# mvisionai/PyGrid

Hardware: AMD Instinct MI355X
Metric: client-diff GB/s aggregated (% of HBM peak) at 1/2/4/8 MI355X; cycle close ms (higher is better)
Workload: dtype f32; 1 GPU; resnet18-fedavg: P_shard=11689512 params/GPU x 1000 clients fp32, resident in HBM; clients=1000, params_per_gpu=11689512, params_total=11689512, parallelism=param-shard1, kernel_variant=0

## Files before the change

### pygrid_amd/csrc/pgh_api.cpp

```cpp
#include <sched.h>

#include <fstream>

#include "pgh_ctx.h"

namespace pgh_detail {

std::vector<int> gpu_local_cpus(int device) {
    std::vector<int> out;
    char bus[64] = {0};
    if (hipDeviceGetPCIBusId(bus, sizeof bus, device) != hipSuccess) { (void)hipGetLastError(); return out; }
    std::string id(bus);
    for (auto& ch : id) ch = (char)std::tolower((unsigned char)ch);
    std::ifstream f("/sys/bus/pci/devices/" + id + "/local_cpulist");
    std::string list;
    if (!f || !std::getline(f, list)) return out;
    cpu_set_t allowed;
    CPU_ZERO(&allowed);
    if (sched_getaffinity(0, sizeof allowed, &allowed) != 0) return out;
    size_t pos = 0;
    while (pos < list.size()) {
        size_t end = list.find(',', pos);
        if (end == std::string::npos) end = list.size();
        const std::string r = list.substr(pos, end - pos);
// ... 105 lines not shown
    *nb = (pg + b - 1) / b;
    int sh = 0;
    while ((int64_t(1) << sh) < b) ++sh;
    *bshift = sh;
}

}

using namespace pgh_detail;

extern "C" {

int pgh_abi_version(void) { return PGH_ABI_VERSION; }

int pgh_device_count(int* n) {
    if (!n) return PGH_E_ARG;
    int k = 0;
    hipError_t e = hipGetDeviceCount(&k);
    if (e != hipSuccess) { *n = 0; return fail(nullptr, PGH_E_HIP, "hipGetDeviceCount: %s", hipGetErrorString(e)); }
    *n = k;
    return PGH_OK;
}

const char* pgh_last_error(const pgh_ctx* ctx) { return ctx ? ctx->err.c_str() : g_create_err.c_str(); }

int pgh_create(int device, size_t pinned_bytes, pgh_ctx** out) {
    if (!out) return fail(nullptr, PGH_E_ARG, "out is NULL");
    *out = nullptr;
    int ndev = 0;
    hipError_t e = hipGetDeviceCount(&ndev);
    if (e != hipSuccess || ndev <= 0) return fail(nullptr, PGH_E_HIP, "no HIP device: %s", hipGetErrorString(e));
    if (device < 0 || device >= ndev) return fail(nullptr, PGH_E_ARG, "device %d out of range [0,%d)", device, ndev);
    auto* c = new pgh_ctx();
    c->device = device;
    DeviceGuard g(device);
    if (pinned_bytes == 0) pinned_bytes = 256ull << 20;
    c->ring.slot_bytes = (pinned_bytes / 2) & ~(size_t)4095;
    if (c->ring.slot_bytes < 4096) c->ring.slot_bytes = 4096;
    c->copy_threads = std::min(16, pgh_int::usable_cpus());
    if (const char* e = std::getenv("PGH_COPY_THREADS")) c->copy_threads = std::max(1, std::atoi(e));
    {
        const char* nu = std::getenv("PGH_NUMA");
        if (!nu || std::atoi(nu) != 0) c->local_cpus = gpu_local_cpus(device);
    }
    c->pool_copy.reset(new CopyPool(c->copy_threads, c->local_cpus));
    if (const char* e = std::getenv("PGH_BLOCK_BYTES")) c->block_bytes = (size_t)std::max(0LL, std::atoll(e));
    if (const char* e = std::getenv("PGH_FINAL_RANGES")) c->final_split = std::max(1, std::atoi(e));
    bool ok = c->stream.make() == hipSuccess && c->copy.make() == hipSuccess && c->aux.make() == hipSuccess;
    ok = ok && xfer_made(c);
    for (pgh_ctx::Event* ev : {&c->copy_done, &c->xsync, &c->aux_ev}) ok = ok && ev->make() == hipSuccess;
    ok = ok && rules_made(c);
    if (!ok) { pgh_destroy(c); return fail(nullptr, PGH_E_HIP, "stream/event creation failed"); }
    {
        bool pin_ok = true;
        auto alloc = [&] {
            bind_thread(c->local_cpus);
            const unsigned flags = c->local_cpus.empty() ? hipHostMallocDefault : hipHostMallocNumaUser;
            for (int k = 0; k < 2 && pin_ok; ++k)
                pin_ok = c->ring.h_pin[k].reserve(c->ring.slot_bytes, flags) ||
                         (flags != hipHostMallocDefault && c->ring.h_pin[k].reserve(c->ring.slot_bytes));
        };
        if (c->local_cpus.empty()) alloc();
        else std::thread([&] { DeviceGuard g2(device); alloc(); }).join();
        if (!pin_ok) {
            const size_t bytes = c->ring.slot_bytes;
            pgh_destroy(c);
            return fail(nullptr, PGH_E_OOM, "pinned host allocation of %zu bytes failed", bytes);
        }
    }
    const char* wu = std::getenv("PGH_WARMUP");
    if (!wu || std::atoi(wu) != 0) {
        const int64_t n = (int64_t)std::min(c->ring.slot_bytes, (size_t)2 << 20) / 8;
        void* d = nullptr;
        ok = hipMalloc(&d, 12 * n) == hipSuccess;
        if (ok) {
            int64_t* d_sum = (int64_t*)d;
            float* d_dec = (float*)((uint8_t*)d + 8 * n);
            void* const pin0 = c->ring.h_pin[0].as<void>();
            std::memset(pin0, 0, 8 * n);
            ok = hipMemcpyAsync(d_sum, pin0, 8 * n, hipMemcpyHostToDevice, c->copy) == hipSuccess &&
                 hipStreamSynchronize(c->copy) == hipSuccess &&
                 (!c->d2h.s || (hipMemcpyAsync(d_sum, pin0, 8 * n, hipMemcpyHostToDevice, c->d2h.s) == hipSuccess &&
                                hipStreamSynchronize(c->d2h.s) == hipSuccess)) &&
                 pgh::launch_secagg_decode(d_sum, d_dec, n, 1.0f, c->stream) == hipSuccess &&
                 hipMemcpyAsync(c->ring.h_pin[1].as<void>(), d_sum, 8 * n, hipMemcpyDeviceToHost, c->stream) == hipSuccess &&
                 hipStreamSynchronize(c->stream) == hipSuccess;
            (void)hipFree(d);
        }
        if (!ok) {
            (void)hipGetLastError();
            (void)hipStreamSynchronize(c->copy);
            (void)hipStreamSynchronize(c->stream);
            c->warmup_skipped = true;
        }
    }
    *out = c;
    return PGH_OK;
}

void pgh_destroy(pgh_ctx* c) {
    if (!c) return;
    if (c->grp) { pgh_group_api::destroy(c); return; }
    DeviceGuard g(c->device);
    sync_work(c);
    if (c->d2h.s) (void)hipStreamSynchronize(c->d2h.s);
    delete c;
}

int pgh_set_layout(pgh_ctx* c, int n_tensors, const int64_t* numel) {
    if (c && c->grp) return pgh_group_api::set_layout(c, n_tensors, numel);
    if (!c) return PGH_E_ARG;
    if (n_tensors <= 0 || !numel) return fail(c, PGH_E_ARG, "need at least one tensor");
    int64_t P = 0;
    for (int k = 0; k < n_tensors; ++k) {
        if (numel[k] < 0) return fail(c, PGH_E_ARG, "tensor %d has negative numel", k);
        P += numel[k];
    }
    if (P <= 0) return fail(c, PGH_E_ARG, "model has no parameters");
    DeviceGuard g(c->device);
    free_slab(c);
    c->numel.assign(numel, numel + n_tensors);
    c->P = P;
    c->layout = true;
    return pgh_set_shard(c, 0, P);
}

int pgh_set_shard(pgh_ctx* c, int64_t lo, int64_t hi) {
    if (c && c->grp) return pgh_group_api::set_shard(c, lo, hi);
    if (!c) return PGH_E_ARG;
    return pgh_detail::set_shard(c, lo, hi, false);
}

}

int pgh_detail::set_shard(pgh_ctx* c, int64_t lo, int64_t hi, bool keep_opt) {
    if (!c->layout) return fail(c, PGH_E_STATE, "pgh_set_layout has not been called");
    if (lo < 0 || hi > c->P || lo >= hi)
        return fail(c, PGH_E_ARG, "shard [%lld,%lld) outside [0,%lld)", (long long)lo, (long long)hi, (long long)c->P);
    DeviceGuard g(c->device);
    free_slab(c);
    const int64_t pvec = std::max((hi - lo + 63) & ~(int64_t)63, (c->vec_min + 63) & ~(int64_t)63);
    rules_shard_set(c, lo, hi, pvec, keep_opt);
    c->lo = lo;
    c->hi = hi;
    c->pg = hi - lo;
    c->pvec = pvec;
    c->st.p_shard = c->pg;
    return PGH_OK;
// ... 184 lines not shown
```

### pygrid_amd/csrc/pgh_host.cpp

```cpp
#include "pgh_host.h"

#include <emmintrin.h>
#include <pthread.h>
#include <sched.h>
#include <sys/mman.h>
#include <unistd.h>

#include <cfloat>
#include <cmath>
#include <cstdlib>
#include <cstring>
#include <fstream>
#include <string>

namespace pgh_detail {

void copy_stream(uint8_t* dst, const uint8_t* src, size_t n) {
    if (n < (256u << 10)) { std::memcpy(dst, src, n); return; }
    const size_t head = (16 - (reinterpret_cast<uintptr_t>(dst) & 15)) & 15;
    std::memcpy(dst, src, head);
    dst += head; src += head; n -= head;
    size_t i = 0;
    for (; i + 64 <= n; i += 64) {
        const __m128i a = _mm_loadu_si128(reinterpret_cast<const __m128i*>(src + i));
        const __m128i b = _mm_loadu_si128(reinterpret_cast<const __m128i*>(src + i + 16));
        const __m128i c = _mm_loadu_si128(reinterpret_cast<const __m128i*>(src + i + 32));
        const __m128i d = _mm_loadu_si128(reinterpret_cast<const __m128i*>(src + i + 48));
        _mm_stream_si128(reinterpret_cast<__m128i*>(dst + i), a);
        _mm_stream_si128(reinterpret_cast<__m128i*>(dst + i + 16), b);
        _mm_stream_si128(reinterpret_cast<__m128i*>(dst + i + 32), c);
        _mm_stream_si128(reinterpret_cast<__m128i*>(dst + i + 48), d);
    }
    std::memcpy(dst + i, src + i, n - i);
    _mm_sfence();
}

void bind_thread(const std::vector<int>& cpus) {
    if (cpus.empty()) return;
    cpu_set_t set;
    CPU_ZERO(&set);
    for (int c : cpus)
        if (c >= 0 && c < CPU_SETSIZE) CPU_SET(c, &set);
    (void)pthread_setaffinity_np(pthread_self(), sizeof set, &set);
}

void scatter_out(const uint8_t* src, size_t off, size_t len, const std::vector<OutPiece>& pieces, CopyPool& pool) {
    std::vector<CopyPool::Seg> segs;
    size_t base = 0;
    for (auto& p : pieces) {
        const size_t a = std::max(off, base), b = std::min(off + len, base + p.n);
        if (a < b) segs.push_back({p.dst + (a - base), src + (a - off), b - a});
        base += p.n;
        if (base >= off + len) break;
    }
    pool.run(segs);
}

void prefault_small(uint8_t* p, size_t n) {
#ifndef MADV_POPULATE_WRITE
#define MADV_POPULATE_WRITE 23
#endif
    if (!p || n == 0 || n >= (4u << 20)) return;
    static const uintptr_t page = (uintptr_t)sysconf(_SC_PAGESIZE);
    const uintptr_t a = (uintptr_t)p & ~(page - 1), b = ((uintptr_t)p + n + page - 1) & ~(page - 1);
    (void)madvise((void*)a, b - a, MADV_POPULATE_WRITE);
}

void prefault_small_any(uint8_t* p, size_t n) {
    static const uintptr_t page = (uintptr_t)sysconf(_SC_PAGESIZE);
    const uintptr_t a = (uintptr_t)p & ~(page - 1), b = ((uintptr_t)p + n + page - 1) & ~(page - 1);
    (void)madvise((void*)a, b - a, MADV_POPULATE_WRITE);
}

bool all_resident(uintptr_t a, uintptr_t b, uintptr_t page) {
    std::vector<unsigned char> v((size_t)((b - a) / page));
    if (v.empty() || mincore((void*)a, b - a, v.data()) != 0) return false;
    for (unsigned char x : v)
        if (!(x & 1)) return false;
    return true;
}

void prefault_parallel(uint8_t* p, size_t n, CopyPool& pool) {
    if (!p || n == 0) return;
    if (n < (4u << 20)) { prefault_small(p, n); return; }
    static const uintptr_t page = (uintptr_t)sysconf(_SC_PAGESIZE);
    const uintptr_t a = (uintptr_t)p & ~(page - 1), b = ((uintptr_t)p + n + page - 1) & ~(page - 1);
    if (all_resident(a, b, page)) return;
    const int k = pool.threads();
    const uintptr_t per = ((b - a) / k + page - 1) & ~(page - 1);
    pool.run_items(k, true, [&](int i) {
        const uintptr_t lo = a + per * (uintptr_t)i, hi = std::min(b, lo + per);
        if (lo < hi) (void)madvise((void*)lo, hi - lo, MADV_POPULATE_WRITE);
    });
}


void philox4x32_10(const uint32_t ctr[4], const uint32_t key[2], uint32_t out[4]) {
    uint32_t c0 = ctr[0], c1 = ctr[1], c2 = ctr[2], c3 = ctr[3], k0 = key[0], k1 = key[1];
    for (int r = 0; r < 10; ++r) {
        const uint64_t p0 = (uint64_t)0xD2511F53u * c0, p1 = (uint64_t)0xCD9E8D57u * c2;
        const uint32_t n0 = (uint32_t)(p1 >> 32) ^ c1 ^ k0, n2 = (uint32_t)(p0 >> 32) ^ c3 ^ k1;
        c1 = (uint32_t)p1;
        c3 = (uint32_t)p0;
        c0 = n0;
        c2 = n2;
        k0 += 0x9E3779B9u;
        k1 += 0xBB67AE85u;
    }
// ... 211 lines not shown
```

### pygrid_amd/csrc/pgh_host.h

```cpp
#pragma once
#include <algorithm>
#include <condition_variable>
#include <cstddef>
#include <cstdint>
#include <functional>
#include <mutex>
#include <thread>
#include <vector>

namespace pgh_int { int usable_cpus(); }

namespace pgh_detail {

void copy_stream(uint8_t* dst, const uint8_t* src, size_t n);
void bind_thread(const std::vector<int>& cpus);

class CopyPool {
  public:
    struct Seg {
        uint8_t* dst;
        const uint8_t* src;
        size_t n;
    };
    explicit CopyPool(int threads, std::vector<int> cpus = {}) : nthreads_(std::max(1, threads)) {
        for (int t = 1; t < nthreads_; ++t)
            workers_.emplace_back([this, t, cpus] {
                bind_thread(cpus);
                loop(t);
            });
    }
    ~CopyPool() {
        {
            std::lock_guard<std::mutex> lk(m_);
            stop_ = true;
            ++gen_;
        }
        cv_.notify_all();
        for (auto& w : workers_) w.join();
    }
    int threads() const { return nthreads_; }
    void run(const std::vector<Seg>& segs) {
        size_t total = 0;
        for (auto& sg : segs) total += sg.n;
        if (total < (4u << 20) || nthreads_ == 1) { copy_range(segs, 0, total); return; }
        {
            std::lock_guard<std::mutex> lk(m_);
            segs_ = &segs;
            total_ = total;
            pending_ = nthreads_ - 1;
            ++gen_;
        }
        cv_.notify_all();
        copy_range(segs, 0, share(total, 0));
        std::unique_lock<std::mutex> lk(m_);
        done_cv_.wait(lk, [this] { return pending_ == 0; });
        segs_ = nullptr;
    }

    void run_items(int n, bool parallel, const std::function<void(int)>& f) {
        if (!parallel || nthreads_ == 1 || n < 2) { for (int i = 0; i < n; ++i) f(i); return; }
        const int per = (n + nthreads_ - 1) / nthreads_;
        std::function<void(int)> job = [&](int t) {
            for (int i = t * per; i < std::min(n, (t + 1) * per); ++i) f(i);
        };
        {
            std::lock_guard<std::mutex> lk(m_);
            fn_ = &job;
            pending_ = nthreads_ - 1;
            ++gen_;
        }
        cv_.notify_all();
        job(0);
        std::unique_lock<std::mutex> lk(m_);
        done_cv_.wait(lk, [this] { return pending_ == 0; });
        fn_ = nullptr;
    }

  private:
    size_t share(size_t total, int t) const {
        const size_t per = ((total + nthreads_ - 1) / nthreads_ + 4095) & ~(size_t)4095;
        return std::min(total, per * (size_t)(t + 1));
    }
    static void copy_range(const std::vector<Seg>& segs, size_t a, size_t b) {
        size_t base = 0;
        for (auto& sg : segs) {
            const size_t lo = std::max(a, base), hi = std::min(b, base + sg.n);
            if (lo < hi) copy_stream(sg.dst + (lo - base), sg.src + (lo - base), hi - lo);
            base += sg.n;
            if (base >= b) break;
        }
    }
    void loop(int t) {
        uint64_t seen = 0;
        for (;;) {
            const std::vector<Seg>* segs;
            const std::function<void(int)>* fn;
            size_t total;
// ... 1 lines not shown
                std::unique_lock<std::mutex> lk(m_);
                cv_.wait(lk, [&] { return gen_ != seen; });
                seen = gen_;
                if (stop_) return;
                segs = segs_;
                fn = fn_;
                total = total_;
            }
            if (fn) {
                (*fn)(t);
            } else {
                const size_t a = t == 0 ? 0 : share(total, t - 1);
                copy_range(*segs, std::min(a, total), share(total, t));
            }
            std::lock_guard<std::mutex> lk(m_);
            if (--pending_ == 0) done_cv_.notify_one();
        }
    }
    int nthreads_;
    std::vector<std::thread> workers_;
    std::mutex m_;
    std::condition_variable cv_, done_cv_;
    const std::vector<Seg>* segs_ = nullptr;
    const std::function<void(int)>* fn_ = nullptr;
    size_t total_ = 0;
    int pending_ = 0;
    uint64_t gen_ = 0;
    bool stop_ = false;
};

struct Piece {
    const uint8_t* src;
    size_t n;
};
struct OutPiece {
    uint8_t* dst;
    size_t n;
};
struct PieceCursor {
    const std::vector<Piece>& pieces;
    size_t pi = 0, poff = 0;
    size_t take(uint8_t* dst, size_t room, std::vector<CopyPool::Seg>* segs) {
        size_t fill = 0;
        while (fill < room && pi < pieces.size()) {
            const size_t m = std::min(pieces[pi].n - poff, room - fill);
            segs->push_back({dst + fill, pieces[pi].src + poff, m});
            fill += m;
            poff += m;
            if (poff == pieces[pi].n) { ++pi; poff = 0; }
        }
        return fill;
    }
};
void scatter_out(const uint8_t* src, size_t off, size_t len, const std::vector<OutPiece>& pieces, CopyPool& pool);

constexpr size_t D2H_PIECE = 8u << 20;
constexpr int64_t INGEST_CHUNK = (int64_t)(D2H_PIECE / 4);
inline int ingest_chunks(int64_t pg) { return (int)((pg + INGEST_CHUNK - 1) / INGEST_CHUNK); }
inline void ingest_chunk_bytes(int64_t pg, int k, size_t* a, size_t* b) {
    *a = (size_t)k * INGEST_CHUNK * 4;
    *b = std::min((size_t)pg * 4, (size_t)(k + 1) * INGEST_CHUNK * 4);
}
inline int64_t ingest_chunk_room(int64_t at) { return (at / INGEST_CHUNK + 1) * INGEST_CHUNK - at; }

void prefault_small_any(uint8_t* p, size_t n);
void prefault_parallel(uint8_t* p, size_t n, CopyPool& pool);

void philox4x32_10(const uint32_t ctr[4], const uint32_t key[2], uint32_t out[4]);
double dp_plog(double s);
void dp_pair_normals(uint64_t key, uint32_t round, uint64_t pair, double* z0, double* z1);
void dp_normals(uint64_t key, uint32_t round, int64_t i0, int64_t n, double* out);
inline double dp_sigma(float z, float c, int64_t n) { return ((double)z * (double)c) / (double)n; }

bool geomed_step(const double* D, int64_t n, float nu, float* w, float* W, double* objective, float* max_w);

int krum_select(const double* D, int n, int f, int m, int32_t* picked, int* n_picked, double* scores);

double row_dot_host(const float* x, const float* y, int64_t p);

int trust_weights(double s0, const double* sumsq, const double* dot, int64_t n, float* w, int32_t* included,
                  int64_t* n_included, double* T, int64_t* n_trusted, float* max_w);

struct SlotCache {
    enum : uint8_t { NONE = 0, QUEUED = 1, VALID = 2 };
    std::vector<uint8_t> state;
    std::vector<double> value;
    std::vector<int32_t> queued;

    double at(int slot) const { return value[(size_t)slot]; }
    bool anything_queued() const { return !queued.empty(); }
    void reserved(int slots) {
        state.assign((size_t)slots, (uint8_t)NONE);
        value.assign((size_t)slots, 0.0);
        queued.clear();
    }
    void written(int slot, int n) { std::fill_n(state.begin() + slot, n, (uint8_t)NONE); }
    std::vector<int32_t> missing(const int32_t* slots, int n) {
        std::vector<int32_t> todo;
        for (int k = 0; k < n; ++k)
            if (state[(size_t)slots[k]] == NONE) {
                todo.push_back(slots[k]);
                state[(size_t)slots[k]] = QUEUED;
            }
        for (int32_t sl : todo) state[(size_t)sl] = NONE;
        return todo;
    }
    void mark_queued(const std::vector<int32_t>& todo) {
        for (int32_t sl : todo) {
            state[(size_t)sl] = QUEUED;
            queued.push_back(sl);
        }
    }
    void harvest(const double* host_image) {
        for (int32_t sl : queued)
            if (state[(size_t)sl] == QUEUED) {
                value[(size_t)sl] = host_image[sl];
// ... 18 lines not shown
```

### pygrid_amd/csrc/pgh_slots.cpp

```cpp
#include "pgh_ctx.h"

using namespace pgh_detail;



namespace {
int slot_fold(pgh_ctx* c, int mode, const int32_t* slots, int n, bool final) {
    RC(check_dtype(c, PGH_F32));
    if (c->streaming) return fail(c, PGH_E_STATE, "context is streaming: slot folds need a RESIDENT slab");
    if (n < 0 || (n > 0 && !slots)) return fail(c, PGH_E_ARG, "bad slot list (n=%d)", n);
    if (c->slot_mode >= 0 && c->slot_mode != mode)
        return fail(c, PGH_E_STATE, "averaging mode changed from %d to %d within a cycle", c->slot_mode, mode);
    RC(check_slot_list(c, slots, n, true));
    const char* const one_fold = rules_one_fold_cycle(mode);
    if (one_fold && c->folded > 0)
        return fail(c, PGH_E_STATE, "%s closes a cycle without earlier slot folds (%lld diffs folded)", one_fold, (long long)c->folded);
    const bool median = mode == PGH_MEDIAN;
    const int64_t c0 = c->folded, total = c0 + n;
    FinalArgs fa;
    fa.ckpt = c->d_ckpt.as<float>();
    fa.out = c->d_out.as<float>();
    if (final) {
        RC(check_ckpt(c, "pgh_fold_slots_finish_resident"));
        if (total == 0) return fail(c, PGH_E_STATE, "no diffs folded");
        RC(fedavg_divisor(c, mode, total, &fa.divisor));
    } else if (n == 0) {
        return PGH_OK;
    }
    DeviceGuard g(c->device);
    const hipStream_t s = c->stream;
    const bool may_range = final && n > 0 && n <= pgh::ROWTAB_MAX && c->pg >= (1 << 20) && c->ranged.valid(c->pg);
    const int32_t* const all_slots = slots;
    const int n_all = n;
    FoldPlan plan;
    RC(rules_slot_plan(c, mode, slots, n, c0, &plan));
    slots = plan.slots;
    n = plan.n;
    if (plan.has_divisor) fa.divisor = plan.divisor;
    const bool ranged = may_range && !plan.whole_rows;
    if (!ranged) RC(order_after_ingest(c, s));
    else if (hipEvent_t dec = c->vdec.last_decode()) CK(c, hipStreamWaitEvent(s, dec, 0));
    if (n > 0) RC(fold_prepare(c, mode, plan.total, s));
    if (median && n > pgh::ROWTAB_MAX) RC(median_row_table(c, slots, n, s));
    int done = 0;
    bool prequeued = false;
    do {
        const int m = median ? n : std::min(n - done, pgh::ROWTAB_MAX);
        pgh::RowTab tab;
        for (int k = 0; k < std::min(m, pgh::ROWTAB_MAX); ++k) tab.rows[k] = slots[done + k] * c->parties;
        const bool first = (c0 + done == 0), last = (done + m == n);
        const int flags = (first ? pgh::FL_FIRST : 0) | (final && last ? pgh::FL_FINAL : 0);
        FoldRows rows{c->d_slab.as<float>(), m};
        if (m <= pgh::ROWTAB_MAX) rows.src.tab = &tab;
        else rows.src.d_rows = median_rows(c);
        const int64_t RF = (int64_t)(D2H_PIECE / 8);
        const int K = (flags & pgh::FL_FINAL) && c->pg >= (1 << 20) ? (int)((c->pg + RF - 1) / RF) : 1;
        if (flags & pgh::FL_FINAL) clear_final_marks(c);
        D2HRing& pre = c->d2h.pre;
        bool prequeue = false;
        if (K > 1 && (flags & pgh::FL_FINAL)) {
            RC(d2h_ring_begin(c, &pre, c->d_out.as<uint8_t>(), 4 * (size_t)c->pg, s, true, false));
            prequeue = pre.base || pre.n_free > 0;
        }
        for (int r = 0; r < K; ++r) {
            const hipStream_t rs = s;
            const int64_t lo = std::min(c->pg, RF * r), hi = K == 1 ? c->pg : std::min(c->pg, RF * (r + 1));
            if (ranged && K > 1) RC(c->ranged.wait_range(c, rs, lo, hi));
            else if (ranged && r == 0) RC(c->ranged.wait_all(c, rs));
            fa.off = lo;
            fa.len = hi - lo;
            RC(fold_launch(c, mode, rows, c0 + done, flags, fa, rs));
            if (K > 1 && (hi % (2 * RF) == 0 || hi == c->pg)) {
                RC(add_final_mark(c, rs, hi));
                if (prequeue) RC(c->d2h.issue_pre(c));
            }
        }
        prequeued = prequeued || prequeue;
        done += m;
    } while (done < n);
    RC(record_fold(c, c->fold_evs, s));
    RC(record_slot_fold(c, all_slots, n_all));
    for (int k = 0; k < n_all; ++k) c->slot_client[(size_t)all_slots[k]] = -1;
    c->folded = total;
    c->st.n_folded = total;
    c->slot_mode = mode;
    if (final) {
        std::swap(c->d_ckpt, c->d_out);
        c->d2h.keep_pre(prequeued, c->d_ckpt.as<uint8_t>());
        c->folded = 0;
        c->slot_mode = -1;
        rules_cycle_finished(c, mode);
    }
    return PGH_OK;
}
}

int pgh_fold_slots(pgh_ctx* c, int mode, const int32_t* slots, int n) {
    if (c) RC(check_mode_use(c, mode, USE_SLOT_EARLY));
    if (c && c->grp) return pgh_group_api::fold_slots(c, mode, slots, n, false);
    if (!c) return PGH_E_ARG;
    return slot_fold(c, mode, slots, n, false);
}

int pgh_fold_slots_finish_resident(pgh_ctx* c, int mode, const int32_t* slots, int n) {
    if (c) RC(check_mode_use(c, mode, USE_SLOT_FINAL));
    if (c && c->grp) return pgh_group_api::fold_slots(c, mode, slots, n, true);
    if (!c) return PGH_E_ARG;
    const double t0 = now_ms();
    RC(slot_fold(c, mode, slots, n, true));
    c->st.close_ms_last = now_ms() - t0;
    return PGH_OK;
}

namespace {
int check_slot_folds(pgh_ctx* c) {
    RC(check_dtype(c, PGH_F32));
    if (c->streaming) return fail(c, PGH_E_STATE, "context is streaming: slot folds need a RESIDENT slab");
    return PGH_OK;
}
}

int pgh_fold_slots_restart(pgh_ctx* c) {
    if (c && c->grp) return pgh_group_api::fold_restart(c);
    if (!c) return PGH_E_ARG;
    RC(check_slot_folds(c));
// ... 8 lines not shown
```

### pygrid_amd/csrc/pgh_xfer.cpp

```cpp
#include "pgh_ctx.h"

namespace pgh_detail {

int h2d_range(pgh_ctx* c, const Dest& d, int64_t i0, const uint8_t* src, int64_t n, hipStream_t s,
              size_t src_room) {
    const size_t es = d.es;
    if (n <= 0) return PGH_OK;
    c->ranged.copy_issued();
    if (d.map.bshift == 62) {
        CK(c, hipMemcpyAsync(d.base + (size_t)i0 * es, src, (size_t)n * es, hipMemcpyHostToDevice, s));
        return PGH_OK;
    }
    const int64_t bw = d.map.ld, i1 = i0 + n;
    int64_t i = i0;
    if (i & (bw - 1)) {
        const int64_t e = std::min(i1, (i | (bw - 1)) + 1);
        CK(c, hipMemcpyAsync(d.base + (size_t)d.map.at(i) * es, src, (size_t)(e - i) * es, hipMemcpyHostToDevice, s));
        src += (size_t)(e - i) * es;
        i = e;
    }
    int64_t full = (i1 - i) / bw;
    const int64_t rest = (i1 - i) - full * bw;
    const bool pad = rest > 0 && d.len > 0 && i1 == d.len && src_room >= (size_t)(bw - rest) * es;
    if (pad) ++full;
    if (full > 0) {
        CK(c, hipMemcpy2DAsync(d.base + (size_t)d.map.at(i) * es, (size_t)d.map.bstride * es, src, (size_t)bw * es,
                               (size_t)bw * es, (size_t)full, hipMemcpyHostToDevice, s));
        src += (size_t)(full * bw) * es;
        i = std::min(i1, i + full * bw);
    }
    if (i < i1)
        CK(c, hipMemcpyAsync(d.base + (size_t)d.map.at(i) * es, src, (size_t)(i1 - i) * es, hipMemcpyHostToDevice, s));
    return PGH_OK;
}

bool is_pinned(const void* p) {
    hipPointerAttribute_t attr;
    if (hipPointerGetAttributes(&attr, p) != hipSuccess) { (void)hipGetLastError(); return false; }
    return attr.type == hipMemoryTypeHost;
}

bool xfer_made(pgh_ctx* c) {
    if (const char* e = std::getenv("PGH_PINNED_GATHER")) c->gather.on = std::atoi(e) != 0;
    if (const char* e = std::getenv("PGH_D2H_STREAM")) c->d2h.mode = std::max(0, std::min(1, std::atoi(e)));
    c->d2h.own = c->d2h.mode > 0;
    bool ok = !c->d2h.own || c->d2h.s.make() == hipSuccess;
    for (Event* ev : {&c->ring.ev[0], &c->ring.ev[1], &c->gather.tab.ev, &c->gather.dma_ev, &c->vdec.tab.ev,
                      &c->vdec.in, &c->vdec.buf[0].done, &c->vdec.buf[1].done})
        ok = ok && ev->make() == hipSuccess;
    return ok;
}

int StagingRing::take(pgh_ctx* c, int* slot) {
    *slot = next;
    next ^= 1;
    if (used[*slot]) CK(c, hipEventSynchronize(ev[*slot]));
    c->d2h.drop_pre();
    return PGH_OK;
}

int StagingRing::poll_free(pgh_ctx* c, int out[2], int* n) {
    for (int k = 0; k < 2; ++k) {
        if (used[k]) {
            const hipError_t q = hipEventQuery(ev[k]);
            if (q == hipErrorNotReady) continue;
            CK(c, q);
            used[k] = false;
        }
        out[(*n)++] = k;
    }
    return PGH_OK;
}

int StagingRing::wait_all(pgh_ctx* c) {
    for (int k = 0; k < 2; ++k) {
        CK(c, hipEventSynchronize(ev[k]));
        used[k] = false;
    }
    return PGH_OK;
}

int HostTable::upload(pgh_ctx* c, void* dev_dst, const void* src, size_t bytes, hipStream_t s) {
    if (used) CK(c, hipEventSynchronize(ev));
    if (bytes > h.cap()) {
        if (!h.reserve(bytes)) return fail(c, PGH_E_OOM, "%s of %zu bytes failed", what, bytes);
        used = false;
    }
    std::memcpy(h.as<void>(), src, bytes);
    c->ranged.copy_issued();
    CK(c, hipMemcpyAsync(dev_dst, h.as<void>(), bytes, hipMemcpyHostToDevice, s));
    CK(c, hipEventRecord(ev, s));
    used = true;
    return PGH_OK;
}

int RangedIngest::begin(pgh_ctx* c, int64_t pg, int* K) {
    *K = chunks(pg);
    if (!c->ev_pool.fill(ev, (size_t)*K)) return fail(c, PGH_E_HIP, "hipEventCreate failed");
    return PGH_OK;
}

int RangedIngest::wait_range(pgh_ctx* c, hipStream_t s, int64_t lo, int64_t hi) {
    for (int64_t k = lo / INGEST_CHUNK; k <= (hi - 1) / INGEST_CHUNK; ++k) CK(c, hipStreamWaitEvent(s, ev[(size_t)k], 0));
// ... 7 lines not shown

int stage_pieces_h2d_ranged(pgh_ctx* c, const Dest& dst, const std::vector<Piece>& pieces, size_t total) {
    H2DTimer t(c);
    int K = 0, slot = 0;
    RC(c->ranged.begin(c, c->pg, &K));
    RC(c->ring.take(c, &slot));
    uint8_t* const pin = c->ring.at(slot);
    PieceCursor cur{pieces};
    for (int k = 0; k < K; ++k) {
        size_t a, b;
        ingest_chunk_bytes(c->pg, k, &a, &b);
        std::vector<CopyPool::Seg> segs;
        cur.take(pin + a, b - a, &segs);
        c->pool_copy->run(segs);
        RC(h2d_range(c, dst, (int64_t)(a / 4), pin + a, (int64_t)((b - a) / 4), c->copy,
                     b == total ? c->ring.slot_bytes - b : 0));
        RC(c->ranged.mark(c, k));
    }
    RC(c->ring.sent(c, slot, c->copy));
    c->ranged.commit(K);
    return t.done(total, total);
}

int stage_pieces_h2d(pgh_ctx* c, const Dest& dst, const std::vector<Piece>& pieces) {
    H2DTimer t(c);
    size_t total = 0, done = 0;
    for (auto& p : pieces) total += p.n;
    PieceCursor cur{pieces};
    while (done < total) {
        int slot = 0;
        RC(c->ring.take(c, &slot));
        std::vector<CopyPool::Seg> segs;
        const size_t fill = cur.take(c->ring.at(slot), c->ring.slot_bytes, &segs);
        c->pool_copy->run(segs);
        RC(h2d_range(c, dst, (int64_t)(done / dst.es), c->ring.at(slot), (int64_t)(fill / dst.es), c->copy,
                     c->ring.slot_bytes - fill));
        RC(c->ring.sent(c, slot, c->copy));
        done += fill;
    }
    return t.done(total, total);
}

int stage_h2d(pgh_ctx* c, const Dest& dst, const uint8_t* src, size_t n, bool pinned_src) {
    if (!pinned_src) return stage_pieces_h2d(c, dst, {Piece{src, n}});
    H2DTimer t(c);
    RC(h2d_range(c, dst, 0, src, (int64_t)(n / dst.es), c->copy));
    CK(c, hipStreamSynchronize(c->copy));
    return t.done(n);
}

static int ensure_d2h_cells(pgh_ctx* c, size_t bytes) {
    if (c->d2h.h.cap() >= bytes) return PGH_OK;
    CK(c, hipStreamSynchronize(c->d2h.s));
    if (!c->d2h.h.reserve(bytes)) return fail(c, PGH_E_OOM, "page-locked D2H cells of %zu bytes failed", bytes);
    return PGH_OK;
}

int d2h_ring_begin(pgh_ctx* c, D2HRing* r, const uint8_t* src, size_t total, hipStream_t s, bool piped, bool may_wait) {
    *r = D2HRing{};
    r->src = src;
    r->total = total;
    r->piped = piped;
    if (piped && c->d2h.own) {
        r->piece = D2H_PIECE;
        r->n_pieces = (total + r->piece - 1) / r->piece;
        RC(ensure_d2h_cells(c, std::min(r->n_pieces, D2H_OWN_CELLS) * r->piece));
        r->base = c->d2h.h.as<uint8_t>();
        r->cells = c->d2h.h.cap() / r->piece;
        r->per_slot = r->cells;
        r->s = c->d2h.s;
        if (!c->ev_pool.fill(c->d2h.ev, std::min(r->cells, r->n_pieces)))
            return fail(c, PGH_E_HIP, "hipEventCreate failed");
        return PGH_OK;
    }
    r->s = piped ? c->copy : s;
    r->piece = std::min(c->ring.slot_bytes, D2H_PIECE);
    r->per_slot = c->ring.slot_bytes / r->piece;
    RC(c->ring.poll_free(c, r->free_slot, &r->n_free));
    if (r->n_free == 0 && !may_wait) return PGH_OK;
    if (r->n_free == 0) {
        RC(c->ring.wait_all(c));
        r->n_free = 2;
    }
    r->cells = (size_t)r->n_free * r->per_slot;
    r->n_pieces = (total + r->piece - 1) / r->piece;
    if (!c->ev_pool.fill(c->d2h.ev, std::min(r->cells, r->n_pieces))) return fail(c, PGH_E_HIP, "hipEventCreate failed");
    return PGH_OK;
}

static uint8_t* d2h_cell(const pgh_ctx* c, const D2HRing& r, size_t j) {
    if (r.base) return r.base + (j % r.cells) * r.piece;
    return c->ring.at(r.free_slot[(j % r.cells) / r.per_slot]) + (j % r.per_slot) * r.piece;
}

static int d2h_piece_ready(pgh_ctx* c, const D2HRing& r, size_t j, bool wait, bool* ready) {
    *ready = true;
    if (!r.piped) return PGH_OK;
    const size_t off = j * r.piece, len = std::min(r.piece, r.total - off);
    const int64_t first = (int64_t)(off / 4), last = (int64_t)((off + len + 3) / 4);
    int64_t start = 0;
    for (auto& m : c->final_marks) {
        if (start >= last) break;
        if (m.end > first) {
            if (wait) {
                CK(c, hipEventSynchronize(m.ev));
            } else {
                const hipError_t q = hipEventQuery(m.ev);
                if (q == hipErrorNotReady) { *ready = false; return PGH_OK; }
                CK(c, q);
            }
        }
        start = m.end;
    }
    return PGH_OK;
}

static int d2h_issue(pgh_ctx* c, D2HRing* r) {
    const size_t j = r->queued, off = j * r->piece, len = std::min(r->piece, r->total - off);
    CK(c, hipMemcpyAsync(d2h_cell(c, *r, j), r->src + off, len, hipMemcpyDeviceToHost, r->s));
    c->st.d2h_bytes_total += len;
    CK(c, hipEventRecord(c->d2h.ev[j % r->cells], r->s));
    ++r->queued;
    return PGH_OK;
}

static int d2h_issue_ready(pgh_ctx* c, D2HRing* r) {
    while (r->queued < r->n_pieces && r->queued < r->done + r->cells) {
        bool ok = false;
        RC(d2h_piece_ready(c, *r, r->queued, false, &ok));
        if (!ok) break;
        RC(d2h_issue(c, r));
    }
    return PGH_OK;
}

int stage_d2h_pieces(pgh_ctx* c, const uint8_t* src, const std::vector<OutPiece>& pieces, hipStream_t s,
                     const std::function<void()>& overlap, bool marks) {
    size_t total = 0;
    for (auto& p : pieces) total += p.n;
    if (total == 0) return PGH_OK;
    const bool piped = marks && !c->final_marks.empty();
    D2HRing r;
    if (piped && c->d2h.adopts(src, total)) {
        r = c->d2h.pre;
    } else {
        RC(d2h_ring_begin(c, &r, src, total, s, piped));
    }
    c->d2h.drop_pre();
    auto copy_out = [&](size_t j) {
        const size_t off = j * r.piece, len = std::min(r.piece, total - off);
        scatter_out(d2h_cell(c, r, j), off, len, pieces, *c->pool_copy);
    };
    const int rc = [&]() -> int {
        if (!piped) {
            while (r.queued < r.n_pieces && r.queued < r.cells) RC(d2h_issue(c, &r));
            if (overlap) overlap();
            for (; r.done < r.n_pieces; ++r.done) {
                CK(c, hipEventSynchronize(c->d2h.ev[r.done % r.cells]));
                copy_out(r.done);
                if (r.queued < r.n_pieces) RC(d2h_issue(c, &r));
            }
        } else {
            RC(d2h_issue_ready(c, &r));
            if (r.queued == r.done) {
                bool ok = false;
                RC(d2h_piece_ready(c, r, r.queued, true, &ok));
                RC(d2h_issue(c, &r));
            }
            if (overlap) overlap();
            while (r.done < r.n_pieces) {
                RC(d2h_issue_ready(c, &r));
                if (r.done < r.queued) {
                    const hipError_t q = hipEventQuery(c->d2h.ev[r.done % r.cells]);
                    if (q == hipSuccess) {
                        copy_out(r.done++);
                        continue;
                    }
                    if (q != hipErrorNotReady) CK(c, q);
                    std::this_thread::yield();
                } else {
                    bool ok = false;
                    RC(d2h_piece_ready(c, r, r.queued, true, &ok));
                    RC(d2h_issue(c, &r));
                }
            }
        }
        return PGH_OK;
    }();
    if (rc != PGH_OK) (void)hipStreamSynchronize(r.s);
    for (int k = 0; k < r.n_free; ++k) c->ring.release(r.free_slot[k]);
    return rc;
}

int D2HState::issue_pre(pgh_ctx* c) {
    const size_t before = pre.queued;
    RC(d2h_issue_ready(c, &pre));
    if (pre.queued > before)
        for (int k = 0; k < pre.n_free; ++k) RC(c->ring.sent(c, pre.free_slot[k], pre.s));
    return PGH_OK;
}

int state_shard_spans(pgh_ctx* c, const uint8_t* pb, size_t n, std::vector<std::pair<size_t, size_t>>* out,
                      const char* what) {
    std::vector<pgh_state::Span> spans;
    std::string msg;
    int rc = pgh_state::scan(pb, n, &spans, &msg);
    if (rc) return fail(c, rc, "%s State: %s", what, msg.c_str());
    if (spans.size() != c->numel.size())
        return fail(c, PGH_E_PARSE, "%s State holds %zu tensors, layout has %zu", what, spans.size(), c->numel.size());
    out->clear();
    int64_t off = 0;
    for (size_t t = 0; t < spans.size(); ++t) {
        if (spans[t].count != c->numel[t])
            return fail(c, PGH_E_PARSE, "%s tensor %zu holds %lld floats, layout %lld", what, t,
                        (long long)spans[t].count, (long long)c->numel[t]);
        const int64_t a = std::max(off, c->lo), b = std::min(off + spans[t].count, c->hi);
        if (a < b) out->push_back({spans[t].offset + 4 * (size_t)(a - off), 4 * (size_t)(b - a)});
        off += spans[t].count;
    }
    return PGH_OK;
}

struct HostDma { uintptr_t lo, hi; Event ev; };
std::mutex g_host_mu;
std::vector<std::pair<uintptr_t, uintptr_t>> g_async_blocks;
std::vector<HostDma> g_host_dmas;
// ... 127 lines not shown
```

### pygrid_amd/csrc/pgh_xfer.h

```cpp
#pragma once
#include "pgh_host.h"
#include "pgh_res.h"

struct pgh_ctx;

namespace pgh_detail {

struct StagingRing {
    PinnedBuf h_pin[2];
    size_t slot_bytes = 0;
    Event ev[2];
    bool used[2] = {false, false};
    int next = 0;

    uint8_t* at(int slot) const { return h_pin[slot].as<uint8_t>(); }
    int take(pgh_ctx* c, int* slot);
    int sent(pgh_ctx* c, int slot, hipStream_t s);
    int poll_free(pgh_ctx* c, int out[2], int* n);
    int wait_all(pgh_ctx* c);
    void release(int slot) { used[slot] = false; }
};

struct HostTable {
    const char* what;
    PinnedBuf h;
    Event ev;
    bool used = false;
    explicit HostTable(const char* what_) : what(what_) {}
    int upload(pgh_ctx* c, void* dev_dst, const void* src, size_t bytes, hipStream_t s);
};

struct RangedIngest {
    bool on = false;
    std::vector<hipEvent_t> ev;
    uint64_t copy_ops = 0, seq = ~0ull;
    int n = 0;

    static int chunks(int64_t pg) { return ingest_chunks(pg); }
    void copy_issued() { ++copy_ops; }
    int begin(pgh_ctx* c, int64_t pg, int* K);
    int mark(pgh_ctx* c, int k);
    void commit(int K) { seq = copy_ops; n = K; }
    bool valid(int64_t pg) const { return on && seq == copy_ops && n == chunks(pg); }
    int wait_range(pgh_ctx* c, hipStream_t s, int64_t lo, int64_t hi);
    int wait_all(pgh_ctx* c, hipStream_t s);
};

constexpr size_t D2H_OWN_CELLS = 8;

struct D2HRing {
    const uint8_t* src = nullptr;
    size_t total = 0, piece = 0, per_slot = 0, cells = 0, n_pieces = 0, queued = 0, done = 0;
    int free_slot[2] = {0, 1};
    int n_free = 0;
    hipStream_t s = nullptr;
    bool piped = false;
    uint8_t* base = nullptr;
};

struct D2HState {
    std::vector<hipEvent_t> ev;
    D2HRing pre;
    bool pre_valid = false;
    bool own = true;
    int mode = 1;
    Stream s;
    PinnedBuf h;

    void drop_pre() { pre_valid = false; }
    void keep_pre(bool queued, const void* ckpt) { pre_valid = queued && pre.src == ckpt; }
    bool adopts(const uint8_t* src, size_t total) const { return pre_valid && pre.src == src && pre.total == total; }
    int issue_pre(pgh_ctx* c);
};

struct VarintBuf {
    DeviceBuf bytes;
    DeviceBuf tab;
    Event done;
    bool used = false;
};
struct VarintDecode {
    VarintBuf buf[2];
    int next = 0;
    Stream s;
    Event in;
    hipEvent_t last = nullptr;
    HostTable tab{"pinned chunk table"};

    VarintBuf& take() { VarintBuf& b = buf[next]; next ^= 1; return b; }
    hipEvent_t last_decode() const { return last; }
};

struct PinnedGather {
    bool on = true;
    DeviceBuf d_bytes;
    DeviceBuf d_tab;
    HostTable tab{"gather chunk table"};
    Event dma_ev;
};

bool xfer_made(pgh_ctx* c);

}
```

Measured before the change: 6798 GB/s.

## Ramp D2H piece sizes and pack pieces into staging segments

Replaces fixed 8 MiB D2H pieces with a schedule that starts with small pieces, doubles them up to the max in the middle, and shrinks them again at the end, so the first host copy-out starts sooner and the final tail is shorter. Pieces are packed into ring segments with explicit dependency indices, and final-fold ranges are aligned to the new piece boundaries. Also allocates D2H cells NUMA-local to the GPU, primes the D2H stream even when warmup is skipped, and lowers the parallel copy-out threshold to 2 MiB. This adds more memcpy calls, events and scheduling complexity.

```diff
diff --git a/pygrid_amd/csrc/pgh_api.cpp b/pygrid_amd/csrc/pgh_api.cpp
--- a/pygrid_amd/csrc/pgh_api.cpp
+++ b/pygrid_amd/csrc/pgh_api.cpp
@@ -181,16 +181,8 @@
     ok = ok && rules_made(c);
     if (!ok) { pgh_destroy(c); return fail(nullptr, PGH_E_HIP, "stream/event creation failed"); }
     {
-        bool pin_ok = true;
-        auto alloc = [&] {
-            bind_thread(c->local_cpus);
-            const unsigned flags = c->local_cpus.empty() ? hipHostMallocDefault : hipHostMallocNumaUser;
-            for (int k = 0; k < 2 && pin_ok; ++k)
-                pin_ok = c->ring.h_pin[k].reserve(c->ring.slot_bytes, flags) ||
-                         (flags != hipHostMallocDefault && c->ring.h_pin[k].reserve(c->ring.slot_bytes));
-        };
-        if (c->local_cpus.empty()) alloc();
-        else std::thread([&] { DeviceGuard g2(device); alloc(); }).join();
+        const bool pin_ok = pinned_on_gpu_socket(c, &c->ring.h_pin[0], c->ring.slot_bytes) &&
+                            pinned_on_gpu_socket(c, &c->ring.h_pin[1], c->ring.slot_bytes);
         if (!pin_ok) {
             const size_t bytes = c->ring.slot_bytes;
             pgh_destroy(c);
@@ -209,8 +201,7 @@
             std::memset(pin0, 0, 8 * n);
             ok = hipMemcpyAsync(d_sum, pin0, 8 * n, hipMemcpyHostToDevice, c->copy) == hipSuccess &&
                  hipStreamSynchronize(c->copy) == hipSuccess &&
-                 (!c->d2h.s || (hipMemcpyAsync(d_sum, pin0, 8 * n, hipMemcpyHostToDevice, c->d2h.s) == hipSuccess &&
-                                hipStreamSynchronize(c->d2h.s) == hipSuccess)) &&
+                 c->d2h.prime(d_sum, pin0, 8 * n) &&
                  pgh::launch_secagg_decode(d_sum, d_dec, n, 1.0f, c->stream) == hipSuccess &&
                  hipMemcpyAsync(c->ring.h_pin[1].as<void>(), d_sum, 8 * n, hipMemcpyDeviceToHost, c->stream) == hipSuccess &&
                  hipStreamSynchronize(c->stream) == hipSuccess;
@@ -223,6 +214,7 @@
             c->warmup_skipped = true;
         }
     }
+    c->d2h.prime_alone(c);
     *out = c;
     return PGH_OK;
 }
diff --git a/pygrid_amd/csrc/pgh_host.cpp b/pygrid_amd/csrc/pgh_host.cpp
--- a/pygrid_amd/csrc/pgh_host.cpp
+++ b/pygrid_amd/csrc/pgh_host.cpp
@@ -53,7 +53,7 @@
         base += p.n;
         if (base >= off + len) break;
     }
-    pool.run(segs);
+    pool.run(segs, COPY_OUT_PARALLEL_FROM);
 }
 
 void prefault_small(uint8_t* p, size_t n) {
diff --git a/pygrid_amd/csrc/pgh_host.h b/pygrid_amd/csrc/pgh_host.h
--- a/pygrid_amd/csrc/pgh_host.h
+++ b/pygrid_amd/csrc/pgh_host.h
@@ -39,10 +39,10 @@
         for (auto& w : workers_) w.join();
     }
     int threads() const { return nthreads_; }
-    void run(const std::vector<Seg>& segs) {
+    void run(const std::vector<Seg>& segs, size_t parallel_from = 4u << 20) {
         size_t total = 0;
         for (auto& sg : segs) total += sg.n;
-        if (total < (4u << 20) || nthreads_ == 1) { copy_range(segs, 0, total); return; }
+        if (total < parallel_from || nthreads_ == 1) { copy_range(segs, 0, total); return; }
         {
             std::lock_guard<std::mutex> lk(m_);
             segs_ = &segs;
@@ -150,6 +150,7 @@
         return fill;
     }
 };
+constexpr size_t COPY_OUT_PARALLEL_FROM = 2u << 20;
 void scatter_out(const uint8_t* src, size_t off, size_t len, const std::vector<OutPiece>& pieces, CopyPool& pool);
 
 constexpr size_t D2H_PIECE = 8u << 20;
@@ -160,6 +161,82 @@
     *b = std::min((size_t)pg * 4, (size_t)(k + 1) * INGEST_CHUNK * 4);
 }
 inline int64_t ingest_chunk_room(int64_t at) { return (at / INGEST_CHUNK + 1) * INGEST_CHUNK - at; }
+
+constexpr size_t D2H_EDGE = 4096;
+constexpr size_t D2H_SMALL_PIECE = 2u << 20;
+struct D2HPiece {
+    size_t off, len;
+    size_t cell = 0;
+    size_t after = 0;
+};
+inline size_t d2h_ramp_steps(size_t max_piece, size_t small) {
+    size_t k = 0;
+    for (size_t s = small; s < max_piece; s *= 2) ++k;
+    return k;
+}
+inline std::vector<D2HPiece> d2h_schedule(size_t total, size_t max_piece = D2H_PIECE, size_t small = D2H_SMALL_PIECE) {
+    std::vector<D2HPiece> out;
+    if (total == 0) return out;
+    const size_t big = std::max<size_t>(1, max_piece / D2H_EDGE);
+    const size_t sm = std::min(big, std::max<size_t>(1, small / D2H_EDGE));
+    size_t left = (total + D2H_EDGE - 1) / D2H_EDGE;
+    std::vector<size_t> front, back;
+    if (sm == big || left < 2 * big) {
+        for (; left > 0; left -= std::min(left, big)) front.push_back(std::min(left, big));
+    } else {
+        size_t f = sm, b = sm;
+        for (bool at_front = true; left > 0; at_front = !at_front) {
+            size_t& next = at_front ? f : b;
+            if (left <= next) break;
+            (at_front ? front : back).push_back(next);
+            left -= next;
+            next = std::min(big, next * 2);
+        }
+        size_t* const nb_f = front.size() > 1 || (front.size() == 1 && back.empty()) ? &front.back() : nullptr;
+        size_t* const nb_b = back.size() > 1 ? &back.back() : nullptr;
+        if (left < sm && nb_f && *nb_f + left <= big) *nb_f += left;
+        else if (left < sm && nb_b && *nb_b + left <= big) *nb_b += left;
+        else front.push_back(left);
+    }
+    front.insert(front.end(), back.rbegin(), back.rend());
+    size_t off = 0;
+    for (size_t pages : front) {
+        const size_t len = std::min(pages * D2H_EDGE, total - off);
+        out.push_back({off, len});
+        off += len;
+    }
+    return out;
+}
+inline size_t d2h_place(std::vector<D2HPiece>* pieces, size_t seg, size_t n_seg) {
+    const size_t cap = seg * n_seg;
+    std::vector<size_t> at(pieces->size());
+    size_t pos = 0, i = 0, in_flight = 0;
+    for (size_t j = 0; j < pieces->size(); ++j) {
+        D2HPiece& p = (*pieces)[j];
+        if (pos % seg + p.len > seg) pos = (pos / seg + 1) * seg;
+        at[j] = pos;
+        p.cell = pos % cap;
+        while (i < j && at[i] + cap < pos + p.len) ++i;
+        p.after = i;
+        in_flight = std::max(in_flight, j - i + 1);
+        pos += (p.len + D2H_EDGE - 1) / D2H_EDGE * D2H_EDGE;
+    }
+    return in_flight;
+}
+struct FinalRange {
+    int64_t lo, hi;
+    bool ends_piece;
+};
+inline std::vector<FinalRange> d2h_final_ranges(int64_t pg, size_t small = D2H_SMALL_PIECE) {
+    std::vector<FinalRange> out;
+    for (const D2HPiece& p : d2h_schedule((size_t)pg * 4, D2H_PIECE, small)) {
+        const int64_t lo = (int64_t)(p.off / 4), hi = (int64_t)((p.off + p.len) / 4);
+        const int64_t mid = lo + (int64_t)(D2H_PIECE / 8);
+        if (mid < hi) out.push_back({lo, mid, false});
+        out.push_back({mid < hi ? mid : lo, hi, true});
+    }
+    return out;
+}
 
 void prefault_small_any(uint8_t* p, size_t n);
 void prefault_parallel(uint8_t* p, size_t n, CopyPool& pool);
diff --git a/pygrid_amd/csrc/pgh_slots.cpp b/pygrid_amd/csrc/pgh_slots.cpp
--- a/pygrid_amd/csrc/pgh_slots.cpp
+++ b/pygrid_amd/csrc/pgh_slots.cpp
@@ -53,24 +53,26 @@
         FoldRows rows{c->d_slab.as<float>(), m};
         if (m <= pgh::ROWTAB_MAX) rows.src.tab = &tab;
         else rows.src.d_rows = median_rows(c);
-        const int64_t RF = (int64_t)(D2H_PIECE / 8);
-        const int K = (flags & pgh::FL_FINAL) && c->pg >= (1 << 20) ? (int)((c->pg + RF - 1) / RF) : 1;
+        std::vector<FinalRange> ranges;
+        if ((flags & pgh::FL_FINAL) && c->pg >= (1 << 20)) ranges = d2h_final_ranges(c->pg, c->d2h.small);
+        if (ranges.size() < 2) ranges = {FinalRange{0, c->pg, false}};
+        const int K = (int)ranges.size();
         if (flags & pgh::FL_FINAL) clear_final_marks(c);
         D2HRing& pre = c->d2h.pre;
         bool prequeue = false;
         if (K > 1 && (flags & pgh::FL_FINAL)) {
             RC(d2h_ring_begin(c, &pre, c->d_out.as<uint8_t>(), 4 * (size_t)c->pg, s, true, false));
-            prequeue = pre.base || pre.n_free > 0;
+            prequeue = pre.set_up();
         }
         for (int r = 0; r < K; ++r) {
             const hipStream_t rs = s;
-            const int64_t lo = std::min(c->pg, RF * r), hi = K == 1 ? c->pg : std::min(c->pg, RF * (r + 1));
+            const int64_t lo = ranges[(size_t)r].lo, hi = ranges[(size_t)r].hi;
             if (ranged && K > 1) RC(c->ranged.wait_range(c, rs, lo, hi));
             else if (ranged && r == 0) RC(c->ranged.wait_all(c, rs));
             fa.off = lo;
             fa.len = hi - lo;
             RC(fold_launch(c, mode, rows, c0 + done, flags, fa, rs));
-            if (K > 1 && (hi % (2 * RF) == 0 || hi == c->pg)) {
+            if (K > 1 && ranges[(size_t)r].ends_piece) {
                 RC(add_final_mark(c, rs, hi));
                 if (prequeue) RC(c->d2h.issue_pre(c));
             }
diff --git a/pygrid_amd/csrc/pgh_xfer.cpp b/pygrid_amd/csrc/pgh_xfer.cpp
--- a/pygrid_amd/csrc/pgh_xfer.cpp
+++ b/pygrid_amd/csrc/pgh_xfer.cpp
@@ -44,11 +44,47 @@
     if (const char* e = std::getenv("PGH_PINNED_GATHER")) c->gather.on = std::atoi(e) != 0;
     if (const char* e = std::getenv("PGH_D2H_STREAM")) c->d2h.mode = std::max(0, std::min(1, std::atoi(e)));
     c->d2h.own = c->d2h.mode > 0;
+    if (const char* e = std::getenv("PGH_D2H_SMALL_PIECE"))
+        c->d2h.small = (size_t)std::max<long long>((long long)D2H_EDGE, std::min<long long>(std::atoll(e), (long long)D2H_PIECE));
     bool ok = !c->d2h.own || c->d2h.s.make() == hipSuccess;
     for (Event* ev : {&c->ring.ev[0], &c->ring.ev[1], &c->gather.tab.ev, &c->gather.dma_ev, &c->vdec.tab.ev,
                       &c->vdec.in, &c->vdec.buf[0].done, &c->vdec.buf[1].done})
         ok = ok && ev->make() == hipSuccess;
     return ok;
+}
+
+bool pinned_on_gpu_socket(pgh_ctx* c, PinnedBuf* buf, size_t bytes) {
+    bool ok = true;
+    auto alloc = [&] {
+        bind_thread(c->local_cpus);
+        const unsigned flags = c->local_cpus.empty() ? hipHostMallocDefault : hipHostMallocNumaUser;
+        ok = buf->reserve(bytes, flags) || (flags != hipHostMallocDefault && buf->reserve(bytes));
+    };
+    if (c->local_cpus.empty()) alloc();
+    else std::thread([&] { DeviceGuard g(c->device); alloc(); }).join();
+    return ok;
+}
+
+bool D2HState::prime(void* dev, const void* pin, size_t bytes) {
+    if (!s) return true;
+    d2h_primed = hipMemcpyAsync(dev, pin, bytes, hipMemcpyHostToDevice, s) == hipSuccess &&
+                 hipStreamSynchronize(s) == hipSuccess;
+    return d2h_primed;
+}
+
+void D2HState::prime_alone(pgh_ctx* c) {
+    if (!s || d2h_primed) return;
+    const size_t bytes = std::min(c->ring.slot_bytes, (size_t)64 << 10);
+    void* d = nullptr;
+    if (hipMalloc(&d, bytes) == hipSuccess) {
+        std::memset(c->ring.at(0), 0, bytes);
+        (void)prime(d, c->ring.at(0), bytes);
+        (void)hipFree(d);
+    }
+    if (!d2h_primed) {
+        (void)hipGetLastError();
+        (void)hipStreamSynchronize(s);
+    }
 }
 
 int StagingRing::take(pgh_ctx* c, int* slot) {
@@ -162,7 +198,14 @@
 static int ensure_d2h_cells(pgh_ctx* c, size_t bytes) {
     if (c->d2h.h.cap() >= bytes) return PGH_OK;
     CK(c, hipStreamSynchronize(c->d2h.s));
-    if (!c->d2h.h.reserve(bytes)) return fail(c, PGH_E_OOM, "page-locked D2H cells of %zu bytes failed", bytes);
+    if (!pinned_on_gpu_socket(c, &c->d2h.h, bytes)) return fail(c, PGH_E_OOM, "page-locked D2H cells of %zu bytes failed", bytes);
+    return PGH_OK;
+}
+
+static int d2h_ring_scheduled(pgh_ctx* c, D2HRing* r, size_t max_piece, size_t n_seg) {
+    r->pieces = d2h_schedule(r->total, max_piece, c->d2h.small);
+    r->n_ev = d2h_place(&r->pieces, r->seg_bytes, n_seg);
+    if (!c->ev_pool.fill(c->d2h.ev, r->n_ev)) return fail(c, PGH_E_HIP, "hipEventCreate failed");
     return PGH_OK;
 }
 
@@ -172,41 +215,29 @@
     r->total = total;
     r->piped = piped;
     if (piped && c->d2h.own) {
-        r->piece = D2H_PIECE;
-        r->n_pieces = (total + r->piece - 1) / r->piece;
-        RC(ensure_d2h_cells(c, std::min(r->n_pieces, D2H_OWN_CELLS) * r->piece));
-        r->base = c->d2h.h.as<uint8_t>();
-        r->cells = c->d2h.h.cap() / r->piece;
-        r->per_slot = r->cells;
+        const size_t whole = (total + D2H_EDGE - 1) / D2H_EDGE * D2H_EDGE;
+        RC(ensure_d2h_cells(c, std::min(whole, D2H_OWN_CELLS * D2H_PIECE)));
+        r->seg[0] = c->d2h.h.as<uint8_t>();
+        r->seg_bytes = c->d2h.h.cap();
         r->s = c->d2h.s;
-        if (!c->ev_pool.fill(c->d2h.ev, std::min(r->cells, r->n_pieces)))
-            return fail(c, PGH_E_HIP, "hipEventCreate failed");
-        return PGH_OK;
+        return d2h_ring_scheduled(c, r, D2H_PIECE, 1);
     }
     r->s = piped ? c->copy : s;
-    r->piece = std::min(c->ring.slot_bytes, D2H_PIECE);
-    r->per_slot = c->ring.slot_bytes / r->piece;
     RC(c->ring.poll_free(c, r->free_slot, &r->n_free));
     if (r->n_free == 0 && !may_wait) return PGH_OK;
     if (r->n_free == 0) {
         RC(c->ring.wait_all(c));
         r->n_free = 2;
     }
-    r->cells = (size_t)r->n_free * r->per_slot;
-    r->n_pieces = (total + r->piece - 1) / r->piece;
-    if (!c->ev_pool.fill(c->d2h.ev, std::min(r->cells, r->n_pieces))) return fail(c, PGH_E_HIP, "hipEventCreate failed");
-    return PGH_OK;
-}
-
-static uint8_t* d2h_cell(const pgh_ctx* c, const D2HRing& r, size_t j) {
-    if (r.base) return r.base + (j % r.cells) * r.piece;
-    return c->ring.at(r.free_slot[(j % r.cells) / r.per_slot]) + (j % r.per_slot) * r.piece;
+    for (int k = 0; k < r->n_free; ++k) r->seg[k] = c->ring.at(r->free_slot[k]);
+    r->seg_bytes = c->ring.slot_bytes;
+    return d2h_ring_scheduled(c, r, std::min(c->ring.slot_bytes, D2H_PIECE), (size_t)r->n_free);
 }
 
 static int d2h_piece_ready(pgh_ctx* c, const D2HRing& r, size_t j, bool wait, bool* ready) {
     *ready = true;
     if (!r.piped) return PGH_OK;
-    const size_t off = j * r.piece, len = std::min(r.piece, r.total - off);
+    const size_t off = r.pieces[j].off, len = r.pieces[j].len;
     const int64_t first = (int64_t)(off / 4), last = (int64_t)((off + len + 3) / 4);
     int64_t start = 0;
     for (auto& m : c->final_marks) {
@@ -222,20 +253,24 @@
         }
         start = m.end;
     }
+    if (start < last) {
+        if (wait) return fail(c, PGH_E_STATE, "D2H piece %zu ends beyond the last range mark", j);
+        *ready = false;
+    }
     return PGH_OK;
 }
 
 static int d2h_issue(pgh_ctx* c, D2HRing* r) {
-    const size_t j = r->queued, off = j * r->piece, len = std::min(r->piece, r->total - off);
-    CK(c, hipMemcpyAsync(d2h_cell(c, *r, j), r->src + off, len, hipMemcpyDeviceToHost, r->s));
-    c->st.d2h_bytes_total += len;
-    CK(c, hipEventRecord(c->d2h.ev[j % r->cells], r->s));
+    const size_t j = r->queued;
+    CK(c, hipMemcpyAsync(r->cell(j), r->src + r->pieces[j].off, r->pieces[j].len, hipMemcpyDeviceToHost, r->s));
+    c->st.d2h_bytes_total += r->pieces[j].len;
+    CK(c, hipEventRecord(c->d2h.ev[j % r->n_ev], r->s));
     ++r->queued;
     return PGH_OK;
 }
 
 static int d2h_issue_ready(pgh_ctx* c, D2HRing* r) {
-    while (r->queued < r->n_pieces && r->queued < r->done + r->cells) {
+    while (r->room()) {
         bool ok = false;
         RC(d2h_piece_ready(c, *r, r->queued, false, &ok));
         if (!ok) break;
@@ -257,18 +292,16 @@
         RC(d2h_ring_begin(c, &r, src, total, s, piped));
     }
     c->d2h.drop_pre();
-    auto copy_out = [&](size_t j) {
-        const size_t off = j * r.piece, len = std::min(r.piece, total - off);
-        scatter_out(d2h_cell(c, r, j), off, len, pieces, *c->pool_copy);
-    };
+    auto copy_out = [&](size_t j) { scatter_out(r.cell(j), r.pieces[j].off, r.pieces[j].len, pieces, *c->pool_copy); };
+    const size_t n_pieces = r.pieces.size();
     const int rc = [&]() -> int {
         if (!piped) {
-            while (r.queued < r.n_pieces && r.queued < r.cells) RC(d2h_issue(c, &r));
+            while (r.room()) RC(d2h_issue(c, &r));
             if (overlap) overlap();
-            for (; r.done < r.n_pieces; ++r.done) {
-                CK(c, hipEventSynchronize(c->d2h.ev[r.done % r.cells]));
-                copy_out(r.done);
-                if (r.queued < r.n_pieces) RC(d2h_issue(c, &r));
+            while (r.done < n_pieces) {
+                CK(c, hipEventSynchronize(c->d2h.ev[r.done % r.n_ev]));
+                copy_out(r.done++);
+                while (r.room()) RC(d2h_issue(c, &r));
             }
         } else {
             RC(d2h_issue_ready(c, &r));
@@ -278,10 +311,10 @@
                 RC(d2h_issue(c, &r));
             }
             if (overlap) overlap();
-            while (r.done < r.n_pieces) {
+            while (r.done < n_pieces) {
                 RC(d2h_issue_ready(c, &r));
                 if (r.done < r.queued) {
-                    const hipError_t q = hipEventQuery(c->d2h.ev[r.done % r.cells]);
+                    const hipError_t q = hipEventQuery(c->d2h.ev[r.done % r.n_ev]);
                     if (q == hipSuccess) {
                         copy_out(r.done++);
                         continue;
diff --git a/pygrid_amd/csrc/pgh_xfer.h b/pygrid_amd/csrc/pgh_xfer.h
--- a/pygrid_amd/csrc/pgh_xfer.h
+++ b/pygrid_amd/csrc/pgh_xfer.h
@@ -50,12 +50,18 @@
 
 struct D2HRing {
     const uint8_t* src = nullptr;
-    size_t total = 0, piece = 0, per_slot = 0, cells = 0, n_pieces = 0, queued = 0, done = 0;
+    size_t total = 0, n_ev = 0, queued = 0, done = 0;
+    std::vector<D2HPiece> pieces;
     int free_slot[2] = {0, 1};
     int n_free = 0;
     hipStream_t s = nullptr;
     bool piped = false;
-    uint8_t* base = nullptr;
+    uint8_t* seg[2] = {nullptr, nullptr};
+    size_t seg_bytes = 0;
+
+    bool set_up() const { return !pieces.empty(); }
+    uint8_t* cell(size_t j) const { return seg[pieces[j].cell / seg_bytes] + pieces[j].cell % seg_bytes; }
+    bool room() const { return queued < pieces.size() && done >= pieces[queued].after; }
 };
 
 struct D2HState {
@@ -66,6 +72,11 @@
     int mode = 1;
     Stream s;
     PinnedBuf h;
+    bool d2h_primed = false;
+    size_t small = D2H_SMALL_PIECE;
+
+    bool prime(void* dev, const void* pin, size_t bytes);
+    void prime_alone(pgh_ctx* c);
 
     void drop_pre() { pre_valid = false; }
     void keep_pre(bool queued, const void* ckpt) { pre_valid = queued && pre.src == ckpt; }
@@ -100,5 +111,6 @@
 };
 
 bool xfer_made(pgh_ctx* c);
+bool pinned_on_gpu_socket(pgh_ctx* c, PinnedBuf* buf, size_t bytes);
 
 }
```

Result: no change. 6801 GB/s, median of 5 (+0.0%).
